# danieldugas/DeepMimic_mujoco

Measured on AMD Instinct MI355X. Metric: env-steps/sec (whole node), 34-DoF humanoid, 4096 envs, at 1/2/4/8 MI355X, higher is better.
Workload: dtype f32

## Files before the change

deepmimic_mujoco_amd/csrc/dm_kernels.hip:

```cpp
#include "../../include/deepmimic_hip.h"
#include "dm_device.h"
#include "dm_rng.h"
#include "dm_topology.h"

#include <math.h>

#include <type_traits>

#define SYNC()                                              \
  do {                                                      \
    __builtin_amdgcn_fence(__ATOMIC_RELEASE, "wavefront");  \
    __builtin_amdgcn_wave_barrier();                        \
    __builtin_amdgcn_fence(__ATOMIC_ACQUIRE, "wavefront");  \
  } while (0)
#define DMK_ENVS_PER_BLOCK 1
#ifndef DMK_WAVES_PER_SIMD
#define DMK_WAVES_PER_SIMD 2
#endif
#ifdef DM_PROFILE
#define PROF_DECL do { if ((threadIdx.x & 63) == 0) { for (int _i = 0; _i < 16; _i++) g_S.prof[_i] = 0; for (int _i = 0; _i < 4; _i++) g_S.prof_stage[_i] = 0; g_S.prof_t = g_S.prof_t0 = __builtin_amdgcn_s_memtime(); } } while (0)
#define PROF_STAGE(i) do { if ((threadIdx.x & 63) == 0 && (i) < 4) g_S.prof_stage[i] = (unsigned)(__builtin_amdgcn_s_memtime() - g_S.prof_t0); } while (0)
#define PROF(i) do { if ((threadIdx.x & 63) == 0) { unsigned long long _t = __builtin_amdgcn_s_memtime(); g_S.prof[i] += (unsigned)(_t - g_S.prof_t); g_S.prof_t = _t; } } while (0)
#if DM_PROFILE == 2
#define PROF2(i) PROF(i)
#else
#define PROF2(i) do {} while (0)
#endif
#else
#define PROF2(i) do {} while (0)
#define PROF_STAGE(i) do {} while (0)
#define PROF_DECL do {} while (0)
#define PROF(i) do {} while (0)
#endif
typedef __attribute__((address_space(3))) const float *lds_cfloat_p;
typedef float lds_f2v __attribute__((ext_vector_type(2)));
typedef float lds_f4v __attribute__((ext_vector_type(4)));
typedef float mfma_f16v __attribute__((ext_vector_type(16)));
#ifndef DMK_MFMA_MIN_ROWS
#define DMK_MFMA_MIN_ROWS 8
#endif
typedef const __attribute__((address_space(1))) DmDev GDev;
typedef const __attribute__((address_space(1))) DmPairDev GPair;
#define MINVALF 1e-15f
#define MAXVALF 1e10f

namespace {

template <int I, int N>
struct StaticFor {
  template <class F>
  static __device__ __forceinline__ void run(F &&f) {
    if constexpr (I < N) {
      if (f(std::integral_constant<int, I>{})) StaticFor<I + 1, N>::run(f);
    }
  }
};

__device__ __forceinline__ float rl(float v, int lane) {
  return __int_as_float(__builtin_amdgcn_readlane(__float_as_int(v), lane));
}
template <unsigned long long MASK>
__device__ __forceinline__ float lane_sel(float a, float b) {
  float out;
  asm("v_cndmask_b32_e64 %0, %1, %2, %3" : "=v"(out) : "v"(b), "v"(a), "s"(MASK));
  return out;
}
template <unsigned long long MASK>
__device__ __forceinline__ int lane_sel_i(int a, int b) {
  int out;
  asm("v_cndmask_b32_e64 %0, %1, %2, %3" : "=v"(out) : "v"(b), "v"(a), "s"(MASK));
  return out;
}
template <int K, int I>
struct ElimAnc {
  static __device__ __forceinline__ void run(float (&C)[DMK_NV], const float Cs) {
    if constexpr (I >= 0) {
      C[I] = fmaf(-rl(Cs, I), C[K], C[I]);
      ElimAnc<K, (I >= 0 ? topo::PARENT[I >= 0 ? I : 0] : -1)>::run(C, Cs);
    }
  }
};
__device__ __forceinline__ float solve_LT(float x, const float dv, const int negdep, const float *M) {
  StaticFor<0, DMK_NV - 1>::run([&](auto ic) {
    constexpr int i = DMK_NV - 1 - decltype(ic)::value;
    const float xi = rl(x * dv, i);
    const float l = lane_sel<topo::anc_mask(i)>(M[topo::MADR[i] + topo::NANC[i] + negdep], 0.f);
    x = fmaf(-l, xi, x);
    return true;
  });
  return x;
}
__device__ __forceinline__ float solve_L(float x, const float dv, const int mrow, const float *M) {
  StaticFor<0, DMK_NV - 1>::run([&](auto jc) {
    constexpr int j = decltype(jc)::value;
    const float xj = rl(x * dv, j);
    const float l = lane_sel<topo::desc_mask(j)>(M[mrow - topo::NANC[j]], 0.f);
    x = fmaf(-l, xj, x);
    return true;
  });
  return x;
}
template <int I, int K = 0>
__device__ __forceinline__ void load_factor_row(lds_cfloat_p Sp, float (&W)[DMK_MAXANC], float &dinv) {
  static_assert(alignof(EnvLds) >= 16 && offsetof(EnvLds, M) % 4 == 0 && offsetof(EnvLds, dinv) % 4 == 0, "EnvLds layout");
  constexpr int n = topo::NANC[I];
  constexpr int a = (int)(offsetof(EnvLds, M) / 4) + topo::MADR[I] + 1 + K;
  if constexpr (K >= n) {
    dinv = Sp[offsetof(EnvLds, dinv) / 4 + I];
  } else if constexpr (a % 4 == 0 && n - K >= 4) {
    const lds_f4v v = *reinterpret_cast<__attribute__((address_space(3))) const lds_f4v *>(Sp + a);
    W[K] = v.x; W[K + 1] = v.y; W[K + 2] = v.z; W[K + 3] = v.w;
    load_factor_row<I, K + 4>(Sp, W, dinv);
  } else if constexpr (a % 2 == 0 && n - K >= 2) {
    const lds_f2v v = *reinterpret_cast<__attribute__((address_space(3))) const lds_f2v *>(Sp + a);
    W[K] = v.x; W[K + 1] = v.y;
    load_factor_row<I, K + 2>(Sp, W, dinv);
  } else {
    W[K] = Sp[a];
    load_factor_row<I, K + 1>(Sp, W, dinv);
  }
}
template <int CTRL>
__device__ __forceinline__ float dpp_mov(float v) {
  return __int_as_float(__builtin_amdgcn_update_dpp(0, __float_as_int(v), CTRL, 0xF, 0xF, true));
}
__device__ __forceinline__ float wave_sum(float v) {
  v += dpp_mov<0xB1>(v);
  v += dpp_mov<0x4E>(v);
  v += dpp_mov<0x141>(v);
  v += dpp_mov<0x140>(v);
  return (rl(v, 0) + rl(v, 16)) + (rl(v, 32) + rl(v, 48));
}
__device__ __forceinline__ unsigned long long lanemask_lt(int lane) {
  return (lane == 0) ? 0ull : (~0ull >> (64 - lane));
}
__device__ __forceinline__ int prefix_count(bool flag, int lane, int *total) {
  unsigned long long m = __ballot(flag);
  *total = __popcll(m);
  return __popcll(m & lanemask_lt(lane));
}

__device__ __forceinline__ void cross3(float *r, const float *a, const float *b) {
  float x = a[1] * b[2] - a[2] * b[1], y = a[2] * b[0] - a[0] * b[2], z = a[0] * b[1] - a[1] * b[0];
  r[0] = x; r[1] = y; r[2] = z;
}
__device__ __forceinline__ float dot3(const float *a, const float *b) {
  return a[0] * b[0] + a[1] * b[1] + a[2] * b[2];
}
__device__ __forceinline__ void quat_mul(float *r, const float *a, const float *b) {
  float w = a[0] * b[0] - a[1] * b[1] - a[2] * b[2] - a[3] * b[3];
  float x = a[0] * b[1] + a[1] * b[0] + a[2] * b[3] - a[3] * b[2];
  float y = a[0] * b[2] - a[1] * b[3] + a[2] * b[0] + a[3] * b[1];
  float z = a[0] * b[3] + a[1] * b[2] - a[2] * b[1] + a[3] * b[0];
  r[0] = w; r[1] = x; r[2] = y; r[3] = z;
}
__device__ __forceinline__ void quat_rot(float *r, const float *q, const float *v) {
  float t[3], u[3];
  cross3(t, q + 1, v);
  t[0] *= 2.f; t[1] *= 2.f; t[2] *= 2.f;
  cross3(u, q + 1, t);
  r[0] = v[0] + q[0] * t[0] + u[0];
  r[1] = v[1] + q[0] * t[1] + u[1];
  r[2] = v[2] + q[0] * t[2] + u[2];
}
// ... 465 lines not shown
    const float Ib[9] = {bi[0], bi[3], bi[4], bi[3], bi[1], bi[5], bi[4], bi[5], bi[2]};
    for (int i = 0; i < 3; i++)
      for (int j = 0; j < 3; j++) Tm[3 * i + j] = R[3 * i] * Ib[j] + R[3 * i + 1] * Ib[3 + j] + R[3 * i + 2] * Ib[6 + j];
    W[0] = Tm[0] * R[0] + Tm[1] * R[1] + Tm[2] * R[2];
    W[1] = Tm[3] * R[3] + Tm[4] * R[4] + Tm[5] * R[5];
    W[2] = Tm[6] * R[6] + Tm[7] * R[7] + Tm[8] * R[8];
    W[3] = Tm[0] * R[3] + Tm[1] * R[4] + Tm[2] * R[5];
    W[4] = Tm[0] * R[6] + Tm[1] * R[7] + Tm[2] * R[8];
    W[5] = Tm[3] * R[6] + Tm[4] * R[7] + Tm[5] * R[8];
    const float o[3] = {S.xipos[lb][0] - com[0], S.xipos[lb][1] - com[1], S.xipos[lb][2] - com[2]};
    const float oo = dot3(o, o);
    float *ci = S.cinert[lb];
    ci[0] = W[0] + bmass * (oo - o[0] * o[0]);
    ci[1] = W[1] + bmass * (oo - o[1] * o[1]);
    ci[2] = W[2] + bmass * (oo - o[2] * o[2]);
    ci[3] = W[3] - bmass * o[0] * o[1];
    ci[4] = W[4] - bmass * o[0] * o[2];
    ci[5] = W[5] - bmass * o[1] * o[2];
    ci[6] = bmass * o[0]; ci[7] = bmass * o[1]; ci[8] = bmass * o[2];
    ci[9] = bmass;
  }
  SYNC();
  PROF(1);
  }
  {
    float acc[10];
    for (int i = 0; i < 10; i++) acc[i] = 0;
    StaticFor<1, DMK_NB>::run([&](auto cc) {
      constexpr int c = decltype(cc)::value;
      const float w = lane_sel<topo::body_ancself_mask(c)>(1.f, 0.f);
#pragma unroll
      for (int i = 0; i < 10; i++) acc[i] = fmaf(w, g_S.cinert[c][i], acc[i]);
      return true;
    });
    if (isbody)
      for (int i = 0; i < 10; i++) S.u.v.crb[lb][i] = acc[i];
  }
  SYNC();
  float C[DMK_NV];
  {
    float cd[6] = {0, 0, 0, 0, 0, 0};
    if (isdof) {
      float buf[6], I[10];
      for (int i = 0; i < 10; i++) I[i] = S.u.v.crb[d_body][i];
      for (int i = 0; i < 6; i++) cd[i] = S.cdof[lk][i];
      mul_inert_vec(buf, I, cd);
      for (int i = 0; i < 6; i++) S.u.v.mbuf[lk][i] = buf[i];
    }
    SYNC();
    const float armv = isdof ? (DAMP2 ? fmaf(T.timestep, T.d_damp[lk], T.d_arm[lk]) : T.d_arm[lk]) : 0.f;
    float dots[DMK_NV];
    {
      const float *bufp = &S.u.v.mbuf[lane & 31][lane >> 5];
      mfma_f16v acc;
#pragma unroll
      for (int v = 0; v < 16; v++) acc[v] = 0.f;
#pragma unroll
      for (int p = 0; p < 3; p++) {
        const auto sw = __builtin_amdgcn_permlane32_swap(__float_as_uint(cd[2 * p]), __float_as_uint(cd[2 * p + 1]), false, false);
        acc = __builtin_amdgcn_mfma_f32_32x32x2f32(bufp[2 * p], __uint_as_float(sw[0]), acc, 0, 0, 0);
      }
#pragma unroll
      for (int v = 0; v < 16; v++) {
        const auto sw = __builtin_amdgcn_permlane32_swap(__float_as_uint(acc[v]), __float_as_uint(acc[v]), false, false);
        dots[(v / 4) * 8 + (v % 4)] = acc[v];
        dots[(v / 4) * 8 + (v % 4) + 4] = __uint_as_float(sw[1]);
      }
#pragma unroll
      for (int k = 32; k < DMK_NV; k++) {
        float d = 0;
#pragma unroll
        for (int i = 0; i < 6; i++) d = fmaf(cd[i], S.u.v.mbuf[k][i], d);
        dots[k] = d;
      }
    }
    StaticFor<0, DMK_NV>::run([&](auto kc) {
      constexpr int k = decltype(kc)::value;
      const float off = lane_sel<topo::anc_mask(k)>(dots[k], 0.f);
      C[k] = lane_sel<(1ull << k)>(dots[k] + armv, off);
      return true;
    });
  }
  PROF(2);
  StaticFor<0, DMK_NV - 1>::run([&](auto ic) {
    constexpr int k = DMK_NV - 1 - decltype(ic)::value;
    const float rk = __builtin_amdgcn_rcpf(rl(C[k], k));
    const float Cs = C[k] * rk;
    ElimAnc<k, topo::PARENT[k]>::run(C, Cs);
    return true;
  });
  const int d_nanc_s = isdof ? d_nanc : 0;
  {
    StaticFor<0, DMK_NV>::run([&](auto kc) {
      constexpr int k = decltype(kc)::value;
      const int real = topo::MADR[k] + topo::NANC[k] - d_nanc_s;
      const int idx = lane_sel_i<(topo::anc_mask(k) | (1ull << k))>(real, DM_NM + 1);
      g_S.M[idx] = C[k];
      return true;
    });
  }
  SYNC();
  float dv = 0.f;
  const int mrow = T.d_madr[lk] + d_nanc;
  const uint64_t ancm = T.d_ancm[lk];
  if (isdof) {
    const float Md = S.M[T.d_madr[lk]];
    dv = 1.0f / Md;
    S.dinv[lk] = dv;
    S.dsqrtinv[lk] = 1.0f / sqrtf(Md);
  }
  SYNC();
  PROF(3);
  float xs = 0;
  if constexpr (DAMP2) {
    xs = isdof ? rhs : 0.f;
  } else {
  if (isbody) {
    float w[6] = {0, 0, 0, 0, 0, 0};
    const int nd = (lb == 1) ? 6 : b_dofnum;
    for (int j = 0; j < 6; j++)
      if (j < nd) {
        const int k = b_dofadr + j;
        const float qv = S.qvel[k];
        for (int i = 0; i < 6; i++) w[i] += S.cdof[k][i] * qv;
      }
    for (int i = 0; i < 6; i++) S.u.v.cacc[lb][i] = w[i];
  }
  SYNC();
  if (isbody) {
    float cv[6] = {0, 0, 0, 0, 0, 0}, u[6] = {0, 0, 0, 0, 0, 0};
#pragma unroll
    for (int c = 0; c < 3; c++) {
      const int cb = (b_chain4 >> (8 * c)) & 0xFF;
      if (cb != 0 && cb != lb)
        for (int i = 0; i < 6; i++) cv[i] += S.u.v.cacc[cb][i];
    }
    if (lb == 1) {
      for (int k = 0; k < 3; k++) {
        const float qv = S.qvel[k];
        for (int i = 0; i < 6; i++) cv[i] += S.cdof[k][i] * qv;
      }
      float dd[3][6];
#pragma unroll
      for (int k = 3; k < 6; k++) {
        float cd[6];
        for (int i = 0; i < 6; i++) cd[i] = S.cdof[k][i];
        cross_motion(dd[k - 3], cv, cd);
      }
#pragma unroll
      for (int k = 3; k < 6; k++) {
        const float qv = S.qvel[k];
        for (int i = 0; i < 6; i++) { u[i] += dd[k - 3][i] * qv; cv[i] += S.cdof[k][i] * qv; }
      }
    } else {
#pragma unroll
      for (int j = 0; j < 3; j++) {
        if (j < b_dofnum) {
          const int k = b_dofadr + j;
          float cd[6], dd[6];
          const float qv = S.qvel[k];
          for (int i = 0; i < 6; i++) cd[i] = S.cdof[k][i];
          cross_motion(dd, cv, cd);
          for (int i = 0; i < 6; i++) { u[i] += dd[i] * qv; cv[i] += cd[i] * qv; }
        }
      }
    }
    for (int i = 0; i < 6; i++) { S.cvel[lb][i] = cv[i]; S.u.v.cfrcsub[lb][i] = u[i]; }
  }
  SYNC();
  PROF2(15);
  if (isbody) {
    float ca[6] = {0, 0, 0, -T.gravity[0], -T.gravity[1], -T.gravity[2]}, cv[6], I[10], f0[6], t0[6], t1[6];
#pragma unroll
// ... 1199 lines not shown
```

deepmimic_mujoco_amd/csrc/dm_topology.h:

```cpp
#pragma once
namespace topo {
constexpr int NV = 34;
constexpr int NM = 310;
constexpr int PARENT[NV] = {-1, 0, 1, 2, 3, 4, 5, 6, 7, 8, 9, 10, 8, 12, 13, 14, 8, 16, 17, 18, 5, 20, 21, 22, 23, 24, 25, 5, 27, 28, 29, 30, 31, 32};
constexpr int NANC[NV] = {0, 1, 2, 3, 4, 5, 6, 7, 8, 9, 10, 11, 9, 10, 11, 12, 9, 10, 11, 12, 6, 7, 8, 9, 10, 11, 12, 6, 7, 8, 9, 10, 11, 12};
constexpr int MADR[NV] = {0, 1, 3, 6, 10, 15, 21, 28, 36, 45, 55, 66, 78, 88, 99, 111, 124, 134, 145, 157, 170, 177, 185, 194, 204, 215, 227, 240, 247, 255, 264, 274, 285, 297};
constexpr bool is_anc(int j, int i) {
  for (int a = PARENT[i]; a >= 0; a = PARENT[a]) if (a == j) return true;
  return false;
}
constexpr int midx(int i, int j) { return MADR[i] + NANC[i] - NANC[j]; }
constexpr int NB = 14;
constexpr int BPARENT[NB] = {0, 0, 1, 2, 2, 4, 2, 6, 1, 8, 9, 1, 11, 12};
constexpr unsigned long long body_ancself_mask(int c) {
  unsigned long long m = 0;
  for (int b = c; b >= 1; b = BPARENT[b]) m |= 1ull << b;
  return m;
}
constexpr unsigned long long desc_mask(int j) {
  unsigned long long m = 0;
  for (int i = 0; i < NV; i++) if (is_anc(j, i)) m |= 1ull << i;
  return m;
}
constexpr unsigned long long anc_mask(int i) {
  unsigned long long m = 0;
  for (int a = PARENT[i]; a >= 0; a = PARENT[a]) m |= 1ull << a;
  return m;
}
}
```

deepmimic_mujoco_amd/gen_topology.py:

```python
import os

from .model import NV, NBODY, load_model

OUT = os.path.join(os.path.dirname(os.path.abspath(__file__)), "csrc", "dm_topology.h")


def render(model):
    parent = [int(x) for x in model.dof_parent]
    nanc = []
    for k in range(NV):
        n, a = 0, parent[k]
        while a >= 0:
            n += 1
            a = parent[a]
        nanc.append(n)
    madr = [int(x) for x in model.dof_Madr]
    bparent = [int(x) for x in model.body_parent]
    lines = [
        "// GENERATED by deepmimic_mujoco_amd/gen_topology.py from deepmimic_humanoid3d.xml — do not edit.",
        "// Dof tree of the model (reference: mjModel.dof_parentid / dof_Madr of the asset loaded at",
        "// src/deepmimic_env.py:301).  Sparse inertia layout: row i = M(i,i), M(i,parent), M(i,grandparent), ...",
        "#pragma once",
        "namespace topo {",
        "constexpr int NV = %d;" % NV,
        "constexpr int NM = %d;" % (madr[-1] + nanc[-1] + 1),
        "constexpr int PARENT[NV] = {%s};" % ", ".join(map(str, parent)),
        "constexpr int NANC[NV] = {%s};" % ", ".join(map(str, nanc)),
        "constexpr int MADR[NV] = {%s};" % ", ".join(map(str, madr)),
        "constexpr bool is_anc(int j, int i) {  // j is a strict ancestor of i",
        "  for (int a = PARENT[i]; a >= 0; a = PARENT[a]) if (a == j) return true;",
        "  return false;",
        "}",
        "constexpr int midx(int i, int j) { return MADR[i] + NANC[i] - NANC[j]; }  // j ancestor-or-self of i",
        "constexpr int NB = %d;" % NBODY,
        "constexpr int BPARENT[NB] = {%s};  // body tree (body 0 = world)" % ", ".join(map(str, bparent)),
        "constexpr unsigned long long body_ancself_mask(int c) {  // bit b: body b (>= 1) is c or an ancestor of c",
        "  unsigned long long m = 0;",
        "  for (int b = c; b >= 1; b = BPARENT[b]) m |= 1ull << b;",
        "  return m;",
        "}",
        "constexpr unsigned long long desc_mask(int j) {  // bit i: dof i is a strict descendant of j",
        "  unsigned long long m = 0;",
        "  for (int i = 0; i < NV; i++) if (is_anc(j, i)) m |= 1ull << i;",
        "  return m;",
        "}",
        "constexpr unsigned long long anc_mask(int i) {  // bit j: dof j is a strict ancestor of i (= the lanes that own M[i][j])",
        "  unsigned long long m = 0;",
        "  for (int a = PARENT[i]; a >= 0; a = PARENT[a]) m |= 1ull << a;",
        "  return m;",
        "}",
        "}  // namespace topo",
        "",
    ]
    return "\n".join(lines)


OUT_G1 = os.path.join(os.path.dirname(os.path.abspath(__file__)), "csrc", "dm_g1_topology.h")


def render_g1(g):
    parent = [int(x) for x in g.dof_parent]
    madr = [int(x) for x in g.dof_Madr]
    nanc = []
    for k in range(g.nv):
        n, a = 0, parent[k]
        while a >= 0:
            n, a = n + 1, parent[a]
        nanc.append(n)
    return "\n".join([
        "// GENERATED by deepmimic_mujoco_amd/gen_topology.py from deepmimic_unitree_g1.xml — do not edit.",
        "// Dof tree of the Unitree G1 model: with it known at compile time the constraint rows are solved against the sparse",
        "// factor in registers (static indices).  dmg1_create() rejects a model whose dof tree differs.",
        "#pragma once",
        "namespace g1topo {",
        "constexpr int NV = %d;" % g.nv,
        "constexpr int PARENT[NV] = {%s};" % ", ".join(map(str, parent)),
        "constexpr int NANC[NV] = {%s};" % ", ".join(map(str, nanc)),
        "constexpr int MADR[NV] = {%s};" % ", ".join(map(str, madr)),
        "}  // namespace g1topo",
        "",
    ])


def _write(path, txt):
    old = open(path).read() if os.path.exists(path) else None
    if old != txt:
        with open(path, "w") as f:
            f.write(txt)


def main():
    _write(OUT, render(load_model()))
    from . import mjcf
    from .model import ASSET_DIR
    _write(OUT_G1, render_g1(mjcf.compile_mjcf_general(os.path.join(ASSET_DIR, "deepmimic_unitree_g1.xml"))))
    return OUT


if __name__ == "__main__":
    print(main())
```

Baseline: 13.96 million.

## Interleave limb-parallel LDL elimination with batched SGPR broadcasts via generated schedule

Replaces the serial per-column LDL^T elimination, which did one readlane-broadcast then one FMA per ancestor, with a generated static schedule. Independent limbs are eliminated side by side, and up to eight readlane broadcasts are batched and pinned in SGPRs by empty asm fences before their FMAs. The aim is to hide the readlane-to-VALU dependency latency and expose ILP across tree branches. The price is more live SGPRs, a large generated table, and reliance on the compiler honoring the asm fences.

```diff
diff --git a/deepmimic_mujoco_amd/csrc/dm_kernels.hip b/deepmimic_mujoco_amd/csrc/dm_kernels.hip
--- a/deepmimic_mujoco_amd/csrc/dm_kernels.hip
+++ b/deepmimic_mujoco_amd/csrc/dm_kernels.hip
@@ -71,15 +71,32 @@
   asm("v_cndmask_b32_e64 %0, %1, %2, %3" : "=v"(out) : "v"(b), "v"(a), "s"(MASK));
   return out;
 }
-template <int K, int I>
-struct ElimAnc {
-  static __device__ __forceinline__ void run(float (&C)[DMK_NV], const float Cs) {
-    if constexpr (I >= 0) {
-      C[I] = fmaf(-rl(Cs, I), C[K], C[I]);
-      ElimAnc<K, (I >= 0 ? topo::PARENT[I >= 0 ? I : 0] : -1)>::run(C, Cs);
-    }
-  }
-};
+template <int N>
+__device__ __forceinline__ void sgpr_batch(float (&a)[topo::FS_SLOTS]) {
+  static_assert(N >= 1 && N <= 8 && topo::FS_SLOTS == 8, "one asm statement per batch size");
+  if constexpr (N == 1) asm("" : "+s"(a[0]));
+  if constexpr (N == 2) asm("" : "+s"(a[0]), "+s"(a[1]));
+  if constexpr (N == 3) asm("" : "+s"(a[0]), "+s"(a[1]), "+s"(a[2]));
+  if constexpr (N == 4) asm("" : "+s"(a[0]), "+s"(a[1]), "+s"(a[2]), "+s"(a[3]));
+  if constexpr (N == 5) asm("" : "+s"(a[0]), "+s"(a[1]), "+s"(a[2]), "+s"(a[3]), "+s"(a[4]));
+  if constexpr (N == 6) asm("" : "+s"(a[0]), "+s"(a[1]), "+s"(a[2]), "+s"(a[3]), "+s"(a[4]), "+s"(a[5]));
+  if constexpr (N == 7) asm("" : "+s"(a[0]), "+s"(a[1]), "+s"(a[2]), "+s"(a[3]), "+s"(a[4]), "+s"(a[5]), "+s"(a[6]));
+  if constexpr (N == 8) asm("" : "+s"(a[0]), "+s"(a[1]), "+s"(a[2]), "+s"(a[3]), "+s"(a[4]), "+s"(a[5]), "+s"(a[6]), "+s"(a[7]));
+}
+__device__ __forceinline__ void factor_columns(float (&C)[DMK_NV]) {
+  float d[topo::FS_SLOTS], m[topo::FS_SLOTS], rk[DMK_NV], Cs[DMK_NV];
+  StaticFor<0, topo::FS_NOPS>::run([&](auto nc) {
+    constexpr topo::FactorOp o = topo::FACTOR_SCHED[decltype(nc)::value];
+    if constexpr (o.op == topo::FS_DIAG) d[o.slot] = rl(C[o.k], o.k);
+    if constexpr (o.op == topo::FS_RCP) rk[o.k] = __builtin_amdgcn_rcpf(d[o.slot]);
+    if constexpr (o.op == topo::FS_SCALE) Cs[o.k] = C[o.k] * rk[o.k];
+    if constexpr (o.op == topo::FS_BCAST) m[o.slot] = rl(Cs[o.k], o.i);
+    if constexpr (o.op == topo::FS_FMA) C[o.i] = fmaf(-m[o.slot], C[o.k], C[o.i]);
+    if constexpr (o.op == topo::FS_FENCE) sgpr_batch<o.slot>(m);
+    if constexpr (o.op == topo::FS_DFENCE) sgpr_batch<o.slot>(d);
+    return true;
+  });
+}
 __device__ __forceinline__ float solve_LT(float x, const float dv, const int negdep, const float *M) {
   StaticFor<0, DMK_NV - 1>::run([&](auto ic) {
     constexpr int i = DMK_NV - 1 - decltype(ic)::value;
@@ -711,13 +728,7 @@
     });
   }
   PROF(2);
-  StaticFor<0, DMK_NV - 1>::run([&](auto ic) {
-    constexpr int k = DMK_NV - 1 - decltype(ic)::value;
-    const float rk = __builtin_amdgcn_rcpf(rl(C[k], k));
-    const float Cs = C[k] * rk;
-    ElimAnc<k, topo::PARENT[k]>::run(C, Cs);
-    return true;
-  });
+  factor_columns(C);
   const int d_nanc_s = isdof ? d_nanc : 0;
   {
     StaticFor<0, DMK_NV>::run([&](auto kc) {
diff --git a/deepmimic_mujoco_amd/csrc/dm_topology.h b/deepmimic_mujoco_amd/csrc/dm_topology.h
--- a/deepmimic_mujoco_amd/csrc/dm_topology.h
+++ b/deepmimic_mujoco_amd/csrc/dm_topology.h
@@ -27,4 +27,128 @@
   for (int a = PARENT[i]; a >= 0; a = PARENT[a]) m |= 1ull << a;
   return m;
 }
+enum { FS_DIAG, FS_RCP, FS_SCALE, FS_BCAST, FS_FMA, FS_FENCE, FS_DFENCE };
+struct FactorOp { unsigned char op, k, i, slot; };
+constexpr int FS_SLOTS = 8;
+constexpr int FS_NOPS = 707;
+constexpr FactorOp FACTOR_SCHED[FS_NOPS] = {
+  {FS_DIAG, 33, 33, 0}, {FS_DIAG, 26, 26, 1}, {FS_DIAG, 19, 19, 2}, {FS_DIAG, 15, 15, 3}, {FS_DIAG, 11, 11, 4}, {FS_DFENCE, 0, 0, 5},
+  {FS_RCP, 33, 33, 0}, {FS_RCP, 26, 26, 1}, {FS_RCP, 19, 19, 2}, {FS_RCP, 15, 15, 3}, {FS_RCP, 11, 11, 4}, {FS_SCALE, 33, 33, 0},
+  {FS_SCALE, 26, 26, 1}, {FS_SCALE, 19, 19, 2}, {FS_SCALE, 15, 15, 3}, {FS_SCALE, 11, 11, 4}, {FS_BCAST, 33, 32, 0}, {FS_BCAST, 26, 25, 1},
+  {FS_BCAST, 19, 18, 2}, {FS_BCAST, 15, 14, 3}, {FS_BCAST, 11, 10, 4}, {FS_BCAST, 33, 31, 5}, {FS_BCAST, 33, 30, 6}, {FS_BCAST, 33, 29, 7},
+  {FS_FENCE, 0, 0, 8}, {FS_FMA, 33, 32, 0}, {FS_FMA, 26, 25, 1}, {FS_FMA, 19, 18, 2}, {FS_FMA, 15, 14, 3}, {FS_FMA, 11, 10, 4},
+  {FS_FMA, 33, 31, 5}, {FS_FMA, 33, 30, 6}, {FS_FMA, 33, 29, 7}, {FS_DIAG, 32, 32, 0}, {FS_DIAG, 25, 25, 1}, {FS_DIAG, 18, 18, 2},
+  {FS_DIAG, 14, 14, 3}, {FS_DIAG, 10, 10, 4}, {FS_DFENCE, 0, 0, 5}, {FS_BCAST, 33, 28, 0}, {FS_BCAST, 33, 27, 1}, {FS_BCAST, 33, 5, 2},
+  {FS_BCAST, 33, 4, 3}, {FS_BCAST, 33, 3, 4}, {FS_BCAST, 33, 2, 5}, {FS_BCAST, 33, 1, 6}, {FS_BCAST, 33, 0, 7}, {FS_FENCE, 0, 0, 8},
+  {FS_FMA, 33, 28, 0}, {FS_FMA, 33, 27, 1}, {FS_FMA, 33, 5, 2}, {FS_FMA, 33, 4, 3}, {FS_FMA, 33, 3, 4}, {FS_FMA, 33, 2, 5},
+  {FS_FMA, 33, 1, 6}, {FS_FMA, 33, 0, 7}, {FS_RCP, 32, 32, 0}, {FS_RCP, 25, 25, 1}, {FS_RCP, 18, 18, 2}, {FS_RCP, 14, 14, 3},
+  {FS_RCP, 10, 10, 4}, {FS_SCALE, 32, 32, 0}, {FS_SCALE, 25, 25, 1}, {FS_SCALE, 18, 18, 2}, {FS_SCALE, 14, 14, 3}, {FS_SCALE, 10, 10, 4},
+  {FS_BCAST, 26, 24, 0}, {FS_BCAST, 26, 23, 1}, {FS_BCAST, 26, 22, 2}, {FS_BCAST, 26, 21, 3}, {FS_BCAST, 26, 20, 4}, {FS_BCAST, 19, 17, 5},
+  {FS_BCAST, 19, 16, 6}, {FS_BCAST, 15, 13, 7}, {FS_FENCE, 0, 0, 8}, {FS_FMA, 26, 24, 0}, {FS_FMA, 26, 23, 1}, {FS_FMA, 26, 22, 2},
+  {FS_FMA, 26, 21, 3}, {FS_FMA, 26, 20, 4}, {FS_FMA, 19, 17, 5}, {FS_FMA, 19, 16, 6}, {FS_FMA, 15, 13, 7}, {FS_BCAST, 15, 12, 0},
+  {FS_BCAST, 11, 9, 1}, {FS_FENCE, 0, 0, 2}, {FS_FMA, 15, 12, 0}, {FS_FMA, 11, 9, 1}, {FS_BCAST, 32, 31, 0}, {FS_BCAST, 25, 24, 1},
+  {FS_BCAST, 18, 17, 2}, {FS_BCAST, 14, 13, 3}, {FS_BCAST, 10, 9, 4}, {FS_BCAST, 32, 30, 5}, {FS_BCAST, 32, 29, 6}, {FS_BCAST, 32, 28, 7},
+  {FS_FENCE, 0, 0, 8}, {FS_FMA, 32, 31, 0}, {FS_FMA, 25, 24, 1}, {FS_FMA, 18, 17, 2}, {FS_FMA, 14, 13, 3}, {FS_FMA, 10, 9, 4},
+  {FS_FMA, 32, 30, 5}, {FS_FMA, 32, 29, 6}, {FS_FMA, 32, 28, 7}, {FS_DIAG, 31, 31, 0}, {FS_DIAG, 24, 24, 1}, {FS_DIAG, 17, 17, 2},
+  {FS_DIAG, 13, 13, 3}, {FS_DIAG, 9, 9, 4}, {FS_DFENCE, 0, 0, 5}, {FS_BCAST, 32, 27, 0}, {FS_BCAST, 32, 5, 1}, {FS_BCAST, 32, 4, 2},
+  {FS_BCAST, 32, 3, 3}, {FS_BCAST, 32, 2, 4}, {FS_BCAST, 32, 1, 5}, {FS_BCAST, 32, 0, 6}, {FS_BCAST, 25, 23, 7}, {FS_FENCE, 0, 0, 8},
+  {FS_FMA, 32, 27, 0}, {FS_FMA, 32, 5, 1}, {FS_FMA, 32, 4, 2}, {FS_FMA, 32, 3, 3}, {FS_FMA, 32, 2, 4}, {FS_FMA, 32, 1, 5},
+  {FS_FMA, 32, 0, 6}, {FS_FMA, 25, 23, 7}, {FS_RCP, 31, 31, 0}, {FS_RCP, 24, 24, 1}, {FS_RCP, 17, 17, 2}, {FS_RCP, 13, 13, 3},
+  {FS_RCP, 9, 9, 4}, {FS_SCALE, 31, 31, 0}, {FS_SCALE, 24, 24, 1}, {FS_SCALE, 17, 17, 2}, {FS_SCALE, 13, 13, 3}, {FS_SCALE, 9, 9, 4},
+  {FS_BCAST, 25, 22, 0}, {FS_BCAST, 25, 21, 1}, {FS_BCAST, 25, 20, 2}, {FS_BCAST, 18, 16, 3}, {FS_BCAST, 14, 12, 4}, {FS_FENCE, 0, 0, 5},
+  {FS_FMA, 25, 22, 0}, {FS_FMA, 25, 21, 1}, {FS_FMA, 25, 20, 2}, {FS_FMA, 18, 16, 3}, {FS_FMA, 14, 12, 4}, {FS_BCAST, 31, 30, 0},
+  {FS_BCAST, 24, 23, 1}, {FS_BCAST, 17, 16, 2}, {FS_BCAST, 13, 12, 3}, {FS_BCAST, 31, 29, 4}, {FS_BCAST, 31, 28, 5}, {FS_BCAST, 31, 27, 6},
+  {FS_BCAST, 31, 5, 7}, {FS_FENCE, 0, 0, 8}, {FS_FMA, 31, 30, 0}, {FS_FMA, 24, 23, 1}, {FS_FMA, 17, 16, 2}, {FS_FMA, 13, 12, 3},
+  {FS_FMA, 31, 29, 4}, {FS_FMA, 31, 28, 5}, {FS_FMA, 31, 27, 6}, {FS_FMA, 31, 5, 7}, {FS_DIAG, 30, 30, 0}, {FS_DIAG, 23, 23, 1},
+  {FS_DIAG, 16, 16, 2}, {FS_DIAG, 12, 12, 3}, {FS_DFENCE, 0, 0, 4}, {FS_BCAST, 31, 4, 0}, {FS_BCAST, 31, 3, 1}, {FS_BCAST, 31, 2, 2},
+  {FS_BCAST, 31, 1, 3}, {FS_BCAST, 31, 0, 4}, {FS_BCAST, 24, 22, 5}, {FS_BCAST, 24, 21, 6}, {FS_BCAST, 24, 20, 7}, {FS_FENCE, 0, 0, 8},
+  {FS_FMA, 31, 4, 0}, {FS_FMA, 31, 3, 1}, {FS_FMA, 31, 2, 2}, {FS_FMA, 31, 1, 3}, {FS_FMA, 31, 0, 4}, {FS_FMA, 24, 22, 5},
+  {FS_FMA, 24, 21, 6}, {FS_FMA, 24, 20, 7}, {FS_RCP, 30, 30, 0}, {FS_RCP, 23, 23, 1}, {FS_RCP, 16, 16, 2}, {FS_RCP, 12, 12, 3},
+  {FS_SCALE, 30, 30, 0}, {FS_SCALE, 23, 23, 1}, {FS_SCALE, 16, 16, 2}, {FS_SCALE, 12, 12, 3}, {FS_BCAST, 30, 29, 0}, {FS_BCAST, 23, 22, 1},
+  {FS_BCAST, 30, 28, 2}, {FS_BCAST, 30, 27, 3}, {FS_BCAST, 30, 5, 4}, {FS_BCAST, 30, 4, 5}, {FS_BCAST, 30, 3, 6}, {FS_BCAST, 30, 2, 7},
+  {FS_FENCE, 0, 0, 8}, {FS_FMA, 30, 29, 0}, {FS_FMA, 23, 22, 1}, {FS_FMA, 30, 28, 2}, {FS_FMA, 30, 27, 3}, {FS_FMA, 30, 5, 4},
+  {FS_FMA, 30, 4, 5}, {FS_FMA, 30, 3, 6}, {FS_FMA, 30, 2, 7}, {FS_DIAG, 29, 29, 0}, {FS_DIAG, 22, 22, 1}, {FS_DFENCE, 0, 0, 2},
+  {FS_BCAST, 30, 1, 0}, {FS_BCAST, 30, 0, 1}, {FS_BCAST, 23, 21, 2}, {FS_BCAST, 23, 20, 3}, {FS_FENCE, 0, 0, 4}, {FS_FMA, 30, 1, 0},
+  {FS_FMA, 30, 0, 1}, {FS_FMA, 23, 21, 2}, {FS_FMA, 23, 20, 3}, {FS_RCP, 29, 29, 0}, {FS_RCP, 22, 22, 1}, {FS_SCALE, 29, 29, 0},
+  {FS_SCALE, 22, 22, 1}, {FS_BCAST, 29, 28, 0}, {FS_BCAST, 22, 21, 1}, {FS_BCAST, 29, 27, 2}, {FS_BCAST, 29, 5, 3}, {FS_BCAST, 29, 4, 4},
+  {FS_BCAST, 29, 3, 5}, {FS_BCAST, 29, 2, 6}, {FS_BCAST, 29, 1, 7}, {FS_FENCE, 0, 0, 8}, {FS_FMA, 29, 28, 0}, {FS_FMA, 22, 21, 1},
+  {FS_FMA, 29, 27, 2}, {FS_FMA, 29, 5, 3}, {FS_FMA, 29, 4, 4}, {FS_FMA, 29, 3, 5}, {FS_FMA, 29, 2, 6}, {FS_FMA, 29, 1, 7},
+  {FS_DIAG, 28, 28, 0}, {FS_DIAG, 21, 21, 1}, {FS_DFENCE, 0, 0, 2}, {FS_BCAST, 29, 0, 0}, {FS_BCAST, 22, 20, 1}, {FS_FENCE, 0, 0, 2},
+  {FS_FMA, 29, 0, 0}, {FS_FMA, 22, 20, 1}, {FS_RCP, 28, 28, 0}, {FS_RCP, 21, 21, 1}, {FS_SCALE, 28, 28, 0}, {FS_SCALE, 21, 21, 1},
+  {FS_BCAST, 28, 27, 0}, {FS_BCAST, 21, 20, 1}, {FS_BCAST, 28, 5, 2}, {FS_BCAST, 28, 4, 3}, {FS_BCAST, 28, 3, 4}, {FS_BCAST, 28, 2, 5},
+  {FS_BCAST, 28, 1, 6}, {FS_BCAST, 28, 0, 7}, {FS_FENCE, 0, 0, 8}, {FS_FMA, 28, 27, 0}, {FS_FMA, 21, 20, 1}, {FS_FMA, 28, 5, 2},
+  {FS_FMA, 28, 4, 3}, {FS_FMA, 28, 3, 4}, {FS_FMA, 28, 2, 5}, {FS_FMA, 28, 1, 6}, {FS_FMA, 28, 0, 7}, {FS_DIAG, 27, 27, 0},
+  {FS_DIAG, 20, 20, 1}, {FS_DFENCE, 0, 0, 2}, {FS_RCP, 27, 27, 0}, {FS_RCP, 20, 20, 1}, {FS_SCALE, 27, 27, 0}, {FS_SCALE, 20, 20, 1},
+  {FS_BCAST, 27, 5, 0}, {FS_BCAST, 27, 4, 1}, {FS_BCAST, 27, 3, 2}, {FS_BCAST, 27, 2, 3}, {FS_BCAST, 27, 1, 4}, {FS_BCAST, 27, 0, 5},
+  {FS_FENCE, 0, 0, 6}, {FS_FMA, 27, 5, 0}, {FS_FMA, 27, 4, 1}, {FS_FMA, 27, 3, 2}, {FS_FMA, 27, 2, 3}, {FS_FMA, 27, 1, 4},
+  {FS_FMA, 27, 0, 5}, {FS_BCAST, 26, 5, 0}, {FS_BCAST, 26, 4, 1}, {FS_BCAST, 26, 3, 2}, {FS_BCAST, 26, 2, 3}, {FS_BCAST, 26, 1, 4},
+  {FS_BCAST, 26, 0, 5}, {FS_BCAST, 25, 5, 6}, {FS_BCAST, 25, 4, 7}, {FS_FENCE, 0, 0, 8}, {FS_FMA, 26, 5, 0}, {FS_FMA, 26, 4, 1},
+  {FS_FMA, 26, 3, 2}, {FS_FMA, 26, 2, 3}, {FS_FMA, 26, 1, 4}, {FS_FMA, 26, 0, 5}, {FS_FMA, 25, 5, 6}, {FS_FMA, 25, 4, 7},
+  {FS_BCAST, 25, 3, 0}, {FS_BCAST, 25, 2, 1}, {FS_BCAST, 25, 1, 2}, {FS_BCAST, 25, 0, 3}, {FS_BCAST, 24, 5, 4}, {FS_BCAST, 24, 4, 5},
+  {FS_BCAST, 24, 3, 6}, {FS_BCAST, 24, 2, 7}, {FS_FENCE, 0, 0, 8}, {FS_FMA, 25, 3, 0}, {FS_FMA, 25, 2, 1}, {FS_FMA, 25, 1, 2},
+  {FS_FMA, 25, 0, 3}, {FS_FMA, 24, 5, 4}, {FS_FMA, 24, 4, 5}, {FS_FMA, 24, 3, 6}, {FS_FMA, 24, 2, 7}, {FS_BCAST, 24, 1, 0},
+  {FS_BCAST, 24, 0, 1}, {FS_BCAST, 23, 5, 2}, {FS_BCAST, 23, 4, 3}, {FS_BCAST, 23, 3, 4}, {FS_BCAST, 23, 2, 5}, {FS_BCAST, 23, 1, 6},
+  {FS_BCAST, 23, 0, 7}, {FS_FENCE, 0, 0, 8}, {FS_FMA, 24, 1, 0}, {FS_FMA, 24, 0, 1}, {FS_FMA, 23, 5, 2}, {FS_FMA, 23, 4, 3},
+  {FS_FMA, 23, 3, 4}, {FS_FMA, 23, 2, 5}, {FS_FMA, 23, 1, 6}, {FS_FMA, 23, 0, 7}, {FS_BCAST, 22, 5, 0}, {FS_BCAST, 22, 4, 1},
+  {FS_BCAST, 22, 3, 2}, {FS_BCAST, 22, 2, 3}, {FS_BCAST, 22, 1, 4}, {FS_BCAST, 22, 0, 5}, {FS_BCAST, 21, 5, 6}, {FS_BCAST, 21, 4, 7},
+  {FS_FENCE, 0, 0, 8}, {FS_FMA, 22, 5, 0}, {FS_FMA, 22, 4, 1}, {FS_FMA, 22, 3, 2}, {FS_FMA, 22, 2, 3}, {FS_FMA, 22, 1, 4},
+  {FS_FMA, 22, 0, 5}, {FS_FMA, 21, 5, 6}, {FS_FMA, 21, 4, 7}, {FS_BCAST, 21, 3, 0}, {FS_BCAST, 21, 2, 1}, {FS_BCAST, 21, 1, 2},
+  {FS_BCAST, 21, 0, 3}, {FS_BCAST, 20, 5, 4}, {FS_BCAST, 20, 4, 5}, {FS_BCAST, 20, 3, 6}, {FS_BCAST, 20, 2, 7}, {FS_FENCE, 0, 0, 8},
+  {FS_FMA, 21, 3, 0}, {FS_FMA, 21, 2, 1}, {FS_FMA, 21, 1, 2}, {FS_FMA, 21, 0, 3}, {FS_FMA, 20, 5, 4}, {FS_FMA, 20, 4, 5},
+  {FS_FMA, 20, 3, 6}, {FS_FMA, 20, 2, 7}, {FS_BCAST, 20, 1, 0}, {FS_BCAST, 20, 0, 1}, {FS_BCAST, 19, 8, 2}, {FS_BCAST, 19, 7, 3},
+  {FS_BCAST, 19, 6, 4}, {FS_BCAST, 19, 5, 5}, {FS_BCAST, 19, 4, 6}, {FS_BCAST, 19, 3, 7}, {FS_FENCE, 0, 0, 8}, {FS_FMA, 20, 1, 0},
+  {FS_FMA, 20, 0, 1}, {FS_FMA, 19, 8, 2}, {FS_FMA, 19, 7, 3}, {FS_FMA, 19, 6, 4}, {FS_FMA, 19, 5, 5}, {FS_FMA, 19, 4, 6},
+  {FS_FMA, 19, 3, 7}, {FS_BCAST, 19, 2, 0}, {FS_BCAST, 19, 1, 1}, {FS_BCAST, 19, 0, 2}, {FS_BCAST, 18, 8, 3}, {FS_BCAST, 18, 7, 4},
+  {FS_BCAST, 18, 6, 5}, {FS_BCAST, 18, 5, 6}, {FS_BCAST, 18, 4, 7}, {FS_FENCE, 0, 0, 8}, {FS_FMA, 19, 2, 0}, {FS_FMA, 19, 1, 1},
+  {FS_FMA, 19, 0, 2}, {FS_FMA, 18, 8, 3}, {FS_FMA, 18, 7, 4}, {FS_FMA, 18, 6, 5}, {FS_FMA, 18, 5, 6}, {FS_FMA, 18, 4, 7},
+  {FS_BCAST, 18, 3, 0}, {FS_BCAST, 18, 2, 1}, {FS_BCAST, 18, 1, 2}, {FS_BCAST, 18, 0, 3}, {FS_BCAST, 17, 8, 4}, {FS_BCAST, 17, 7, 5},
+  {FS_BCAST, 17, 6, 6}, {FS_BCAST, 17, 5, 7}, {FS_FENCE, 0, 0, 8}, {FS_FMA, 18, 3, 0}, {FS_FMA, 18, 2, 1}, {FS_FMA, 18, 1, 2},
+  {FS_FMA, 18, 0, 3}, {FS_FMA, 17, 8, 4}, {FS_FMA, 17, 7, 5}, {FS_FMA, 17, 6, 6}, {FS_FMA, 17, 5, 7}, {FS_BCAST, 17, 4, 0},
+  {FS_BCAST, 17, 3, 1}, {FS_BCAST, 17, 2, 2}, {FS_BCAST, 17, 1, 3}, {FS_BCAST, 17, 0, 4}, {FS_BCAST, 16, 8, 5}, {FS_BCAST, 16, 7, 6},
+  {FS_BCAST, 16, 6, 7}, {FS_FENCE, 0, 0, 8}, {FS_FMA, 17, 4, 0}, {FS_FMA, 17, 3, 1}, {FS_FMA, 17, 2, 2}, {FS_FMA, 17, 1, 3},
+  {FS_FMA, 17, 0, 4}, {FS_FMA, 16, 8, 5}, {FS_FMA, 16, 7, 6}, {FS_FMA, 16, 6, 7}, {FS_BCAST, 16, 5, 0}, {FS_BCAST, 16, 4, 1},
+  {FS_BCAST, 16, 3, 2}, {FS_BCAST, 16, 2, 3}, {FS_BCAST, 16, 1, 4}, {FS_BCAST, 16, 0, 5}, {FS_BCAST, 15, 8, 6}, {FS_BCAST, 15, 7, 7},
+  {FS_FENCE, 0, 0, 8}, {FS_FMA, 16, 5, 0}, {FS_FMA, 16, 4, 1}, {FS_FMA, 16, 3, 2}, {FS_FMA, 16, 2, 3}, {FS_FMA, 16, 1, 4},
+  {FS_FMA, 16, 0, 5}, {FS_FMA, 15, 8, 6}, {FS_FMA, 15, 7, 7}, {FS_BCAST, 15, 6, 0}, {FS_BCAST, 15, 5, 1}, {FS_BCAST, 15, 4, 2},
+  {FS_BCAST, 15, 3, 3}, {FS_BCAST, 15, 2, 4}, {FS_BCAST, 15, 1, 5}, {FS_BCAST, 15, 0, 6}, {FS_BCAST, 14, 8, 7}, {FS_FENCE, 0, 0, 8},
+  {FS_FMA, 15, 6, 0}, {FS_FMA, 15, 5, 1}, {FS_FMA, 15, 4, 2}, {FS_FMA, 15, 3, 3}, {FS_FMA, 15, 2, 4}, {FS_FMA, 15, 1, 5},
+  {FS_FMA, 15, 0, 6}, {FS_FMA, 14, 8, 7}, {FS_BCAST, 14, 7, 0}, {FS_BCAST, 14, 6, 1}, {FS_BCAST, 14, 5, 2}, {FS_BCAST, 14, 4, 3},
+  {FS_BCAST, 14, 3, 4}, {FS_BCAST, 14, 2, 5}, {FS_BCAST, 14, 1, 6}, {FS_BCAST, 14, 0, 7}, {FS_FENCE, 0, 0, 8}, {FS_FMA, 14, 7, 0},
+  {FS_FMA, 14, 6, 1}, {FS_FMA, 14, 5, 2}, {FS_FMA, 14, 4, 3}, {FS_FMA, 14, 3, 4}, {FS_FMA, 14, 2, 5}, {FS_FMA, 14, 1, 6},
+  {FS_FMA, 14, 0, 7}, {FS_BCAST, 13, 8, 0}, {FS_BCAST, 13, 7, 1}, {FS_BCAST, 13, 6, 2}, {FS_BCAST, 13, 5, 3}, {FS_BCAST, 13, 4, 4},
+  {FS_BCAST, 13, 3, 5}, {FS_BCAST, 13, 2, 6}, {FS_BCAST, 13, 1, 7}, {FS_FENCE, 0, 0, 8}, {FS_FMA, 13, 8, 0}, {FS_FMA, 13, 7, 1},
+  {FS_FMA, 13, 6, 2}, {FS_FMA, 13, 5, 3}, {FS_FMA, 13, 4, 4}, {FS_FMA, 13, 3, 5}, {FS_FMA, 13, 2, 6}, {FS_FMA, 13, 1, 7},
+  {FS_BCAST, 13, 0, 0}, {FS_BCAST, 12, 8, 1}, {FS_BCAST, 12, 7, 2}, {FS_BCAST, 12, 6, 3}, {FS_BCAST, 12, 5, 4}, {FS_BCAST, 12, 4, 5},
+  {FS_BCAST, 12, 3, 6}, {FS_BCAST, 12, 2, 7}, {FS_FENCE, 0, 0, 8}, {FS_FMA, 13, 0, 0}, {FS_FMA, 12, 8, 1}, {FS_FMA, 12, 7, 2},
+  {FS_FMA, 12, 6, 3}, {FS_FMA, 12, 5, 4}, {FS_FMA, 12, 4, 5}, {FS_FMA, 12, 3, 6}, {FS_FMA, 12, 2, 7}, {FS_BCAST, 12, 1, 0},
+  {FS_BCAST, 12, 0, 1}, {FS_BCAST, 11, 8, 2}, {FS_BCAST, 11, 7, 3}, {FS_BCAST, 11, 6, 4}, {FS_BCAST, 11, 5, 5}, {FS_BCAST, 11, 4, 6},
+  {FS_BCAST, 11, 3, 7}, {FS_FENCE, 0, 0, 8}, {FS_FMA, 12, 1, 0}, {FS_FMA, 12, 0, 1}, {FS_FMA, 11, 8, 2}, {FS_FMA, 11, 7, 3},
+  {FS_FMA, 11, 6, 4}, {FS_FMA, 11, 5, 5}, {FS_FMA, 11, 4, 6}, {FS_FMA, 11, 3, 7}, {FS_BCAST, 11, 2, 0}, {FS_BCAST, 11, 1, 1},
+  {FS_BCAST, 11, 0, 2}, {FS_BCAST, 10, 8, 3}, {FS_BCAST, 10, 7, 4}, {FS_BCAST, 10, 6, 5}, {FS_BCAST, 10, 5, 6}, {FS_BCAST, 10, 4, 7},
+  {FS_FENCE, 0, 0, 8}, {FS_FMA, 11, 2, 0}, {FS_FMA, 11, 1, 1}, {FS_FMA, 11, 0, 2}, {FS_FMA, 10, 8, 3}, {FS_FMA, 10, 7, 4},
+  {FS_FMA, 10, 6, 5}, {FS_FMA, 10, 5, 6}, {FS_FMA, 10, 4, 7}, {FS_BCAST, 10, 3, 0}, {FS_BCAST, 10, 2, 1}, {FS_BCAST, 10, 1, 2},
+  {FS_BCAST, 10, 0, 3}, {FS_BCAST, 9, 8, 4}, {FS_BCAST, 9, 7, 5}, {FS_BCAST, 9, 6, 6}, {FS_BCAST, 9, 5, 7}, {FS_FENCE, 0, 0, 8},
+  {FS_FMA, 10, 3, 0}, {FS_FMA, 10, 2, 1}, {FS_FMA, 10, 1, 2}, {FS_FMA, 10, 0, 3}, {FS_FMA, 9, 8, 4}, {FS_FMA, 9, 7, 5},
+  {FS_FMA, 9, 6, 6}, {FS_FMA, 9, 5, 7}, {FS_BCAST, 9, 4, 0}, {FS_BCAST, 9, 3, 1}, {FS_BCAST, 9, 2, 2}, {FS_BCAST, 9, 1, 3},
+  {FS_BCAST, 9, 0, 4}, {FS_FENCE, 0, 0, 5}, {FS_FMA, 9, 4, 0}, {FS_FMA, 9, 3, 1}, {FS_FMA, 9, 2, 2}, {FS_FMA, 9, 1, 3},
+  {FS_FMA, 9, 0, 4}, {FS_DIAG, 8, 8, 0}, {FS_DFENCE, 0, 0, 1}, {FS_RCP, 8, 8, 0}, {FS_SCALE, 8, 8, 0}, {FS_BCAST, 8, 7, 0},
+  {FS_BCAST, 8, 6, 1}, {FS_BCAST, 8, 5, 2}, {FS_BCAST, 8, 4, 3}, {FS_BCAST, 8, 3, 4}, {FS_BCAST, 8, 2, 5}, {FS_BCAST, 8, 1, 6},
+  {FS_BCAST, 8, 0, 7}, {FS_FENCE, 0, 0, 8}, {FS_FMA, 8, 7, 0}, {FS_FMA, 8, 6, 1}, {FS_FMA, 8, 5, 2}, {FS_FMA, 8, 4, 3},
+  {FS_FMA, 8, 3, 4}, {FS_FMA, 8, 2, 5}, {FS_FMA, 8, 1, 6}, {FS_FMA, 8, 0, 7}, {FS_DIAG, 7, 7, 0}, {FS_DFENCE, 0, 0, 1},
+  {FS_RCP, 7, 7, 0}, {FS_SCALE, 7, 7, 0}, {FS_BCAST, 7, 6, 0}, {FS_BCAST, 7, 5, 1}, {FS_BCAST, 7, 4, 2}, {FS_BCAST, 7, 3, 3},
+  {FS_BCAST, 7, 2, 4}, {FS_BCAST, 7, 1, 5}, {FS_BCAST, 7, 0, 6}, {FS_FENCE, 0, 0, 7}, {FS_FMA, 7, 6, 0}, {FS_FMA, 7, 5, 1},
+  {FS_FMA, 7, 4, 2}, {FS_FMA, 7, 3, 3}, {FS_FMA, 7, 2, 4}, {FS_FMA, 7, 1, 5}, {FS_FMA, 7, 0, 6}, {FS_DIAG, 6, 6, 0},
+  {FS_DFENCE, 0, 0, 1}, {FS_RCP, 6, 6, 0}, {FS_SCALE, 6, 6, 0}, {FS_BCAST, 6, 5, 0}, {FS_BCAST, 6, 4, 1}, {FS_BCAST, 6, 3, 2},
+  {FS_BCAST, 6, 2, 3}, {FS_BCAST, 6, 1, 4}, {FS_BCAST, 6, 0, 5}, {FS_FENCE, 0, 0, 6}, {FS_FMA, 6, 5, 0}, {FS_FMA, 6, 4, 1},
+  {FS_FMA, 6, 3, 2}, {FS_FMA, 6, 2, 3}, {FS_FMA, 6, 1, 4}, {FS_FMA, 6, 0, 5}, {FS_DIAG, 5, 5, 0}, {FS_DFENCE, 0, 0, 1},
+  {FS_RCP, 5, 5, 0}, {FS_SCALE, 5, 5, 0}, {FS_BCAST, 5, 4, 0}, {FS_BCAST, 5, 3, 1}, {FS_BCAST, 5, 2, 2}, {FS_BCAST, 5, 1, 3},
+  {FS_BCAST, 5, 0, 4}, {FS_FENCE, 0, 0, 5}, {FS_FMA, 5, 4, 0}, {FS_FMA, 5, 3, 1}, {FS_FMA, 5, 2, 2}, {FS_FMA, 5, 1, 3},
+  {FS_FMA, 5, 0, 4}, {FS_DIAG, 4, 4, 0}, {FS_DFENCE, 0, 0, 1}, {FS_RCP, 4, 4, 0}, {FS_SCALE, 4, 4, 0}, {FS_BCAST, 4, 3, 0},
+  {FS_BCAST, 4, 2, 1}, {FS_BCAST, 4, 1, 2}, {FS_BCAST, 4, 0, 3}, {FS_FENCE, 0, 0, 4}, {FS_FMA, 4, 3, 0}, {FS_FMA, 4, 2, 1},
+  {FS_FMA, 4, 1, 2}, {FS_FMA, 4, 0, 3}, {FS_DIAG, 3, 3, 0}, {FS_DFENCE, 0, 0, 1}, {FS_RCP, 3, 3, 0}, {FS_SCALE, 3, 3, 0},
+  {FS_BCAST, 3, 2, 0}, {FS_BCAST, 3, 1, 1}, {FS_BCAST, 3, 0, 2}, {FS_FENCE, 0, 0, 3}, {FS_FMA, 3, 2, 0}, {FS_FMA, 3, 1, 1},
+  {FS_FMA, 3, 0, 2}, {FS_DIAG, 2, 2, 0}, {FS_DFENCE, 0, 0, 1}, {FS_RCP, 2, 2, 0}, {FS_SCALE, 2, 2, 0}, {FS_BCAST, 2, 1, 0},
+  {FS_BCAST, 2, 0, 1}, {FS_FENCE, 0, 0, 2}, {FS_FMA, 2, 1, 0}, {FS_FMA, 2, 0, 1}, {FS_DIAG, 1, 1, 0}, {FS_DFENCE, 0, 0, 1},
+  {FS_RCP, 1, 1, 0}, {FS_SCALE, 1, 1, 0}, {FS_BCAST, 1, 0, 0}, {FS_FENCE, 0, 0, 1}, {FS_FMA, 1, 0, 0},
+};
 }
diff --git a/deepmimic_mujoco_amd/gen_topology.py b/deepmimic_mujoco_amd/gen_topology.py
--- a/deepmimic_mujoco_amd/gen_topology.py
+++ b/deepmimic_mujoco_amd/gen_topology.py
@@ -3,6 +3,116 @@
 from .model import NV, NBODY, load_model
 
 OUT = os.path.join(os.path.dirname(os.path.abspath(__file__)), "csrc", "dm_topology.h")
+
+FS_DIAG, FS_RCP, FS_SCALE, FS_BCAST, FS_FMA, FS_FENCE, FS_DFENCE = range(7)
+FS_SLOTS = 8
+
+
+def factor_schedule(parent, slots=FS_SLOTS):
+    nv = len(parent)
+    kids = [[c for c in range(nv) if parent[c] == k] for k in range(nv)]
+    anc = []
+    for k in range(nv):
+        a, l = parent[k], []
+        while a >= 0:
+            l.append(a)
+            a = parent[a]
+        anc.append(l)
+    trunk = [k for k in range(nv) if any(len(kids[j]) > 1 for j in range(nv) if j == k or k in anc[j])]
+    limbs = []
+    for k in reversed(range(nv)):
+        if k not in trunk and not kids[k]:
+            limb = [k]
+            while parent[limb[-1]] not in trunk and parent[limb[-1]] >= 0:
+                limb.append(parent[limb[-1]])
+            limbs.append(limb)
+    ops = []
+
+    def heads(ks, stages):
+        for op in stages:
+            for s, k in enumerate(ks):
+                ops.append((op, k, k, s))
+            if op == FS_DIAG and ks:
+                ops.append((FS_DFENCE, 0, 0, len(ks)))
+
+    def batches(pairs):
+        return [pairs[b:b + slots] for b in range(0, len(pairs), slots)]
+
+    def updates(batch):
+        for s, (k, i) in enumerate(batch):
+            ops.append((FS_BCAST, k, i, s))
+        ops.append((FS_FENCE, 0, 0, len(batch)))
+        for s, (k, i) in enumerate(batch):
+            ops.append((FS_FMA, k, i, s))
+
+    first = limbs[0] if limbs and all(min(limbs[0]) > max(l) for l in limbs[1:]) else None
+    assert len(limbs) <= slots
+    rounds = [[l[r] for l in limbs if len(l) > r] for r in range(max((len(l) for l in limbs), default=0))]
+    for r, piv in enumerate(rounds):
+        nxt = rounds[r + 1] if r + 1 < len(rounds) else []
+        if r == 0:
+            heads(piv, (FS_DIAG, FS_RCP, FS_SCALE))
+        own = {k: [i for i in anc[k] if i not in trunk or k in (first or ())] for k in piv}
+        todo = batches([(k, own[k][0]) for k in piv if own[k]] + [(k, i) for k in piv for i in own[k][1:]])
+        for n, batch in enumerate(todo):
+            updates(batch)
+            if n == 0:
+                heads(nxt, (FS_DIAG,))
+            if n == min(1, len(todo) - 1):
+                heads(nxt, (FS_RCP, FS_SCALE))
+    later = sorted((k for l in limbs if l is not first for k in l), reverse=True)
+    for batch in batches([(k, i) for k in later for i in anc[k] if i in trunk]):
+        updates(batch)
+    for k in sorted(trunk, reverse=True):
+        if k >= 1:
+            heads([k], (FS_DIAG, FS_RCP, FS_SCALE))
+            for batch in batches([(k, i) for i in anc[k]]):
+                updates(batch)
+    check_factor_schedule(parent, ops)
+    return ops
+
+
+def check_factor_schedule(parent, ops):
+    nv = len(parent)
+    anc = {k: [] for k in range(nv)}
+    for k in range(nv):
+        a = parent[k]
+        while a >= 0:
+            anc[k].append(a)
+            a = parent[a]
+    pairs = [(k, i) for k in range(nv) for i in anc[k]]
+    fmas = [(k, i) for op, k, i, s in ops if op == FS_FMA]
+    assert sorted(fmas) == sorted(pairs), "the updates are not a permutation of the (dof, ancestor) pairs"
+    for op in (FS_DIAG, FS_RCP, FS_SCALE):
+        assert sorted(k for o, k, i, s in ops if o == op) == list(range(1, nv)), "every dof 1.. has one pivot"
+    last = {i: nv for i in range(nv)}
+    left = {i: sum(1 for p in pairs if p[1] == i) for i in range(nv)}
+    slot, dslot, have = {}, {}, {k: set() for k in range(nv)}
+    for n, (op, k, i, s) in enumerate(ops):
+        if op == FS_DIAG:
+            assert left[k] == 0, "op %d: pivot %d before the last update into C[%d]" % (n, k, k)
+            dslot[s] = (k, False)
+        elif op == FS_RCP:
+            assert dslot.get(s) == (k, True), "op %d: rcp of dof %d reads slot %d, which does not hold its fenced diagonal" % (n, k, s)
+            have[k].add(FS_RCP)
+        elif op == FS_SCALE:
+            assert FS_RCP in have[k], "op %d: scale of dof %d before its rcp" % (n, k)
+            have[k].add(FS_SCALE)
+        elif op == FS_BCAST:
+            assert FS_SCALE in have[k] and i in anc[k], "op %d: broadcast (%d, %d)" % (n, k, i)
+            slot[s] = (k, i, False)
+        elif op == FS_FENCE:
+            for t in range(s):
+                slot[t] = slot[t][:2] + (True,)
+        elif op == FS_DFENCE:
+            for t in range(s):
+                dslot[t] = (dslot[t][0], True)
+        elif op == FS_FMA:
+            assert slot.get(s) == (k, i, True), "op %d: update (%d, %d) reads slot %d, which does not hold its fenced multiplier" % (n, k, i, s)
+            assert k < last[i], "op %d: update (%d, %d) after the update of dof %d into C[%d]" % (n, k, i, last[i], i)
+            last[i] = k
+            left[i] -= 1
+    return True
 
 
 def render(model):
@@ -49,6 +159,22 @@
         "  for (int a = PARENT[i]; a >= 0; a = PARENT[a]) m |= 1ull << a;",
         "  return m;",
         "}",
+    ]
+    sched = factor_schedule(parent)
+    lines += [
+        "// Emission order of the L^T D L elimination in fwd_smooth: a topological order of its dependency DAG in which the",
+        "// limbs run side by side and the broadcasts of a batch precede their FMAs (gen_topology.factor_schedule).",
+        "enum { FS_DIAG, FS_RCP, FS_SCALE, FS_BCAST, FS_FMA, FS_FENCE, FS_DFENCE };",
+        "struct FactorOp { unsigned char op, k, i, slot; };",
+        "constexpr int FS_SLOTS = %d;" % FS_SLOTS,
+        "constexpr int FS_NOPS = %d;" % len(sched),
+        "constexpr FactorOp FACTOR_SCHED[FS_NOPS] = {",
+    ]
+    names = ("FS_DIAG", "FS_RCP", "FS_SCALE", "FS_BCAST", "FS_FMA", "FS_FENCE", "FS_DFENCE")
+    for b in range(0, len(sched), 6):
+        lines.append("  " + " ".join("{%s, %d, %d, %d}," % (names[op], k, i, s) for op, k, i, s in sched[b:b + 6]))
+    lines += [
+        "};",
         "}  // namespace topo",
         "",
     ]
```

Measured after the change: 14.22 million (median of 6 runs). 1.9% higher.
